# UW-RoboSoccer/tsid_control

Measured on NVIDIA B200. Metric: tsid_qp_ticks_per_sec, higher is better.
Workload: dtype f64

## Files before the change

### tsid_control_b200/csrc/tsidb_kernels.cuh

```cuda
#ifndef TSIDB_KERNELS_CUH_
#define TSIDB_KERNELS_CUH_

#include <cstddef>
#include "tsidb_const.h"

#ifndef TSIDB_EMU
#include <cuda_runtime.h>
#define TSIDB_DEV __device__ __forceinline__
#define TSIDB_HD __host__ __device__
#define TSIDB_DEVNI __device__ __noinline__
__constant__ DevConst g_const[TSIDB_MAX_SLOTS];
#endif

#define FULL 0xffffffffu
#define SCHED_FENCE() asm volatile("" ::: "memory")
#ifdef TSIDB_EMU
#define PHASE_SYNC_D() ((void)0)
#define PHASE_SYNC_E() ((void)0)
#else
#define PHASE_SYNC_D() do { if (TSIDB_LOCK_D) __syncthreads(); } while (0)
#define PHASE_SYNC_E() do { if (TSIDB_LOCK_E) __syncthreads(); } while (0)
#endif
#define TS_EPS 2.220446049250313e-16
#define TS_INF 1.7976931348623157e308
// ... 815 lines not shown
#pragma unroll
      for (int k = 0; k < NV; k++) b[k] = JF[(f * 6 + r) * TSIDB_NVX + k];
    } else if (e < neq) {
      const int u = e - ncm;
#pragma unroll
      for (int k = 0; k < NV; k++) b[k] = Mm[u * SM_LDM + k];
#pragma unroll
      for (int s = 0; s < NC; s++) {
        {
          const int f = (s == 0) ? f0 : 1;
          double jf[6];
#pragma unroll
          for (int r = 0; r < 6; r++) jf[r] = JF[(f * 6 + r) * TSIDB_NVX + u];
#pragma unroll
          for (int o = 0; o < 12; o++) {
            double acc = 0.0;
#pragma unroll
            for (int r = 0; r < 6; r++) acc += C.T[r][o] * jf[r];
            b[NV + 12 * s + o] = -acc;
          }
        }
      }
    } else if (e == neq) {
#pragma unroll
      for (int k = 0; k < N; k++) b[k] = gv[k];
    }
    fwdsub_L<NV, NC>(b, L, ild, C);
    if (e == neq) {
#pragma unroll
      for (int k = 0; k < N; k++) b[k] = -b[k];
    }
    PHASE_SYNC_E();
    auto qr_step = [&](const int i, auto top_tag) {
      constexpr bool top = decltype(top_tag)::value;
      PHASE_SYNC_E();
      const int head = top ? i : NV + (i - ncm);
      __syncwarp();
      if (lane == i) {
        double2* c2 = reinterpret_cast<double2*>(colp);
#pragma unroll
        for (int k = (top ? 0 : ncm); k < (top ? NV : N); k += 2) c2[k >> 1] = make_double2(b[k], b[k + 1]);
      }
      __syncwarp();
      double part = 0.0;
      if (top) {
        if (lane > i && lane < NV) { const double t = colp[lane]; part = t * t; }
      } else {
        for (int k = lane; k < n; k += 32) {
          const bool in_span = (k >= ncm && k < NV) || k > head;
          if (in_span) { const double t = colp[k]; part += t * t; }
        }
      }
      const double sigma = warp_sum(part);
      const double alpha = colp[head];
      const double nrm = sqrt(alpha * alpha + sigma);
      const double beta = (alpha >= 0.0) ? -nrm : nrm;
      if (fabs(beta) <= TS_EPS * R_norm && err == ST_OPTIMAL) err = ST_ERROR;
      R_norm = fmax(R_norm, fabs(beta));
      const double uh = alpha - beta;
      if (top) {
        Vt[i * LDV + lane] = (lane == i) ? uh : ((lane > i && lane < NV) ? colp[lane] : 0.0);
        if (lane + 32 < N) Vt[i * LDV + lane + 32] = 0.0;
      } else {
        for (int k = lane; k < N; k += 32) {
          const bool in_span = (k >= ncm && k < NV) || k > head;
          Vt[i * LDV + k] = (k == head) ? uh : (in_span ? colp[k] : 0.0);
        }
      }
      const double tau = -1.0 / (beta * uh);
      if (lane == 0) { tauq[i] = tau; Rd[i] = beta; }
      __syncwarp();
      if (lane > i && lane <= neq) {
        if (top) reflect<N, 0, NV, (NC == 2)>(b, Vt + i * LDV, tau);
        else reflect<N, ncm, N, (NC == 2)>(b, Vt + i * LDV, tau);
      }
    };
    constexpr int n_top = (nc == 0) ? neq : ncm;
    for (int i = 0; i < n_top; i++) qr_step(i, BoolTag<true>());
    for (int i = n_top; i < neq; i++) qr_step(i, BoolTag<false>());
    __syncwarp();
    if (lane <= neq) {
      store_R1<N, NV, ncm, neq>(R1, b, lane);
    }
    if (lane == neq) {
#pragma unroll
      for (int k = 0; k < N; k++) gv[k] = b[k];
    }
    __syncwarp();
  }
  PHASE_SYNC_E();
  {
    double rhs = 0.0;
    if (lane < ncm) {
      const int s = lane / 6, r = lane % 6;
      const int f = (s == 0) ? f0 : 1;
      rhs = bmot[6 * f + r];
    } else if (lane < neq) {
      rhs = -sm[SE_oNle + lane - ncm];
    }
    const double ird = (lane < neq) ? 1.0 / Rd[lane] : 0.0;
    double accv = rhs * ird;
#pragma unroll
    for (int i = 0; i < neq - 1; i++) {
      const double wi = shfl(accv, i);
      if (lane > i && lane < neq) accv -= (R1[i * SM_LDB + lane] * ird) * wi;
    }
    __syncwarp();
    if (lane < neq) gv[(lane < ncm || nc == 0) ? lane : NV + (lane - ncm)] = accv;
    __syncwarp();
  }
  double y0 = (lane < n) ? gv[lane] : 0.0;
  double y1 = (lane + 32 < n) ? gv[lane + 32] : 0.0;
#pragma unroll
  for (int i = neq - 1; i >= 0; i--) {
    const double v0 = (lane < N) ? Vt[i * LDV + lane] : 0.0;
    const double v1 = (i >= ((nc == 0) ? neq : ncm) && lane + 32 < N) ? Vt[i * LDV + lane + 32] : 0.0;
    const double w = tauq[i] * warp_sum(v0 * y0 + v1 * y1);
    y0 -= w * v0;
    y1 -= w * v1;
  }
  w0v[lane] = y0;
  if (lane + 32 < N) w0v[lane + 32] = y1;
  __syncwarp();
  if (lane < 12 * nc) {
    const int s = lane / 12, i = lane % 12;
    double acc0 = 0.0, acc1 = 0.0;
#pragma unroll
    for (int k = 0; k < 12; k += 2) {
      acc0 += lfinv_sm[k * 12 + i] * w0v[NV + 12 * s + k];
      acc1 += lfinv_sm[(k + 1) * 12 + i] * w0v[NV + 12 * s + k + 1];
    }
    x[NV + lane] = acc0 + acc1;
  }
  {
    const double il = (lane < NV) ? ild[lane] : 0.0;
    y0 *= il;
#pragma unroll
    for (int k = NV - 1; k > 0; k--) {
      const double xk = shfl(y0, k);
      if (lane < k) y0 -= (L[k * SM_LDM + lane] * il) * xk;
    }
  }
  if (lane < NV) x[lane] = y0;
  __syncwarp();
  R_norm_out = R_norm;
  return err;
}

#define SA_LDJA 20
#define SA_LDM 26
struct ALayout {
  int n, m, ldj;
  int oSc, oJ2, oMa, oJFa, oNle, oVj, oX, image;
  int oWr, oR, oNP, oD, oBar, per_env;
};
TSIDB_HD constexpr int even_up(int x) { return (x + 1) & ~1; }
TSIDB_HD constexpr ALayout a_layout(int nv, int nc) {
  ALayout L{};
  const int na = nv - 6;
  L.n = nv + 12 * nc;
  L.m = na + 6 * nc;
  L.ldj = (((L.m / 2) & 1) != 0) ? L.m : L.m + 2;
  L.oSc = 0;
  L.oJ2 = 4;
  L.oMa = L.oJ2 + L.n * L.ldj;
  L.oJFa = L.oMa + na * SA_LDM;
  L.oNle = L.oJFa + 6 * nc * SA_LDJA;
  L.oX = L.oNle + even_up(na);
  L.oVj = L.oX + even_up(L.n);
  L.image = L.oVj + even_up(na);
  L.oWr = L.oVj;
  L.oR = L.oWr + 12;
  L.oNP = L.oR + even_up(L.m * (L.m + 1) / 2);
  L.oD = L.oNP + even_up(L.n);
  L.oBar = L.oD + L.m + 2;
  L.per_env = L.oBar + 2;
  if (L.per_env < L.image + 2) L.per_env = L.image + 2;
  return L;
}
template <int NV, int NC>
struct AL {
  enum : int { n = a_layout(NV, NC).n, m = a_layout(NV, NC).m, ldj = a_layout(NV, NC).ldj, oSc = a_layout(NV, NC).oSc, oJ2 = a_layout(NV, NC).oJ2, oMa = a_layout(NV, NC).oMa, oJFa = a_layout(NV, NC).oJFa, oNle = a_layout(NV, NC).oNle, oVj = a_layout(NV, NC).oVj, oX = a_layout(NV, NC).oX, image = a_layout(NV, NC).image, oWr = a_layout(NV, NC).oWr, oR = a_layout(NV, NC).oR, oNP = a_layout(NV, NC).oNP, oD = a_layout(NV, NC).oD, oBar = a_layout(NV, NC).oBar, per_env = a_layout(NV, NC).per_env };
};
#define SA_IMAGE (a_layout(TSIDB_NVX, 2).image)
#define SA_oSc 0
#define TSIDB_AS_WARPS_DS 8
#define TSIDB_AS_WARPS_SS 12
#define TSIDB_AS_WARPS_FL 12

#ifndef TSIDB_EMU
TSIDB_DEV unsigned smem_u32(const void* p) { return (unsigned)__cvta_generic_to_shared(p); }
TSIDB_DEV void mbar_init(void* bar, int count) {
  asm volatile("mbarrier.init.shared::cta.b64 [%0], %1;" ::"r"(smem_u32(bar)), "r"(count) : "memory");
  asm volatile("fence.mbarrier_init.release.cluster;" ::: "memory");
}
TSIDB_DEV void bulk_load(void* dst, const void* src, unsigned bytes, void* bar) {
  asm volatile("fence.proxy.async.shared::cta;" ::: "memory");
  asm volatile("mbarrier.arrive.expect_tx.shared::cta.b64 _, [%0], %1;" ::"r"(smem_u32(bar)), "r"(bytes) : "memory");
  asm volatile("cp.async.bulk.shared::cluster.global.mbarrier::complete_tx::bytes [%0], [%1], %2, [%3];" ::"r"(smem_u32(dst)),
               "l"(src), "r"(bytes), "r"(smem_u32(bar))
               : "memory");
}
TSIDB_DEV void bulk_store(void* dst, const void* src, unsigned bytes) {
  asm volatile("cp.async.bulk.global.shared::cta.bulk_group [%0], [%1], %2;" ::"l"(dst), "r"(smem_u32(src)), "r"(bytes) : "memory");
}
TSIDB_DEV void bulk_store_commit() { asm volatile("cp.async.bulk.commit_group;" ::: "memory"); }
TSIDB_DEV void bulk_store_wait_read() { asm volatile("cp.async.bulk.wait_group.read 0;" ::: "memory"); }
TSIDB_DEV void bulk_prefetch_l2(const void* src, unsigned bytes) {
  asm volatile("cp.async.bulk.prefetch.L2.global [%0], %1;" ::"l"(src), "r"(bytes) : "memory");
}
TSIDB_DEV void mbar_wait(void* bar, unsigned parity) {
  unsigned ok = 0;
  const unsigned addr = smem_u32(bar);
  do {
    asm volatile("{ .reg .pred p; mbarrier.try_wait.parity.shared::cta.b64 p, [%1], %2; selp.u32 %0, 1, 0, p; }"
                 : "=r"(ok)
                 : "r"(addr), "r"(parity)
                 : "memory");
  } while (!ok);
}
#endif

TSIDB_DEV unsigned long long sortable(double v) {
  unsigned long long b;
  memcpy(&b, &v, 8);
  return (b >> 63) ? ~b : (b | 0x8000000000000000ull);
}
struct LaneConst {
  double lb, ub;
  double tmin, tmax;
  double vmin, vmax;
  double fric[3];
  double Trow[12];
};

struct ASCtx {
  int na, nv;
  int ldj;
  double* J2;
  const double* Ma;
  const double* JFa;
  int nfr;
  int wro;
  const double* nle_a;
  const double* vj;
  double* x;
  double* wr;
  double *Rp, *np, *dd;
};

TSIDB_DEV int fvar0(int nv, int mask, int f) { return nv + ((f == 1 && (mask & 1)) ? 12 : 0); }

#define NRM_LANE0 12
TSIDB_DEV int cid_of(int na, int lane, int slot) {
  return slot == 0 ? lane : (slot == 1 ? 32 + lane - NRM_LANE0 : 36 + (slot - 2) * na + lane);
}
TSIDB_DEV void cid_owner(int na, int cid, int& lane, int& slot) {
  if (cid < 32) { lane = cid; slot = 0; }
  else if (cid < 36) { lane = cid - 32 + NRM_LANE0; slot = 1; }
  else { const int k = cid - 36; slot = 2 + k / na; lane = k - (slot - 2) * na; }
}
TSIDB_DEV int cid_bit(int na, int nv, int cid) {
  if (cid < 32) return 34 * (cid >> 4) + 17 + (cid & 15);
  if (cid < 36) return 34 * ((cid - 32) >> 1) + (((cid - 32) & 1) ? 33 : 16);
  if (cid < 36 + 2 * na) { int k = cid - 36; return 68 + k; }
  int k = cid - 36 - 2 * na;
  int side = k >= na ? 1 : 0, i = k - side * na;
  return 68 + 2 * na + side * nv + 6 + i;
}

TSIDB_DEV void lane_const_init(const DevConst& C, LaneConst& K, int lane) {
  const int na = C.na;
#pragma unroll
  for (int j = 0; j < 12; j++) K.Trow[j] = (lane >= NRM_LANE0 && lane < NRM_LANE0 + 4) ? C.nrm[j % 3] : C.T[lane % 6][j];
#pragma unroll
  for (int j = 0; j < 3; j++) K.fric[j] = C.fric[lane & 3][j];
  K.tmin = (lane < na) ? C.tau_min[lane] : 0.0;
  K.tmax = (lane < na) ? C.tau_max[lane] : 0.0;
  K.vmin = (lane < na) ? C.v_min[lane] : 0.0;
  K.vmax = (lane < na) ? C.v_max[lane] : 0.0;
  K.lb = K.ub = 0.0;
}

TSIDB_DEV void lane_const_load(const double* tables, LaneConst& K, int lane) {
  const double* t = tables + TBL_oLANE + lane;
#pragma unroll
  for (int j = 0; j < 12; j++) K.Trow[j] = t[j * 32];
#pragma unroll
  for (int j = 0; j < 3; j++) K.fric[j] = t[(12 + j) * 32];
  K.tmin = t[15 * 32]; K.tmax = t[16 * 32]; K.vmin = t[17 * 32]; K.vmax = t[18 * 32];
  K.lb = K.ub = 0.0;
}

TSIDB_DEV void eval_rows(const DevConst& C, const ASCtx& S, const LaneConst& K, int lane, int mask, double (&s)[6]) {
  const int na = S.na, nv = S.nv;
  const double* x = S.x;
#pragma unroll
  for (int k = 0; k < 6; k++) s[k] = TS_INF;
  {
    const int f = lane >> 4, c = (lane & 15) >> 2;
    if ((mask >> f) & 1) {
      const double* ff = x + fvar0(nv, mask, f) + 3 * c;
      s[0] = -(K.fric[0] * ff[0] + K.fric[1] * ff[1] + K.fric[2] * ff[2]);
    }
  }
  if (lane < 4) {
    const int f = lane >> 1, side = lane & 1;
    if ((mask >> f) & 1) {
      const double* ff = x + fvar0(nv, mask, f);
      double t = 0.0;
#pragma unroll
      for (int c = 0; c < 4; c++) t += C.nrm[0] * ff[3 * c] + C.nrm[1] * ff[3 * c + 1] + C.nrm[2] * ff[3 * c + 2];
      s[1] = side ? (C.fmax - t) : (t - C.fmin);
    }
  }
  if (lane < na) {
    if (C.use_tb) {
      const double2* Mr = reinterpret_cast<const double2*>(S.Ma + lane * SA_LDM);
      const double2* x2 = reinterpret_cast<const double2*>(x);
      double t0 = S.nle_a[lane], t1 = 0.0, t2 = 0.0, t3 = 0.0;
      int j = 0;
      for (; j + 1 < nv / 2; j += 2) {
        const double2 m0 = Mr[j], m1 = Mr[j + 1], x0 = x2[j], x1 = x2[j + 1];
        t0 += m0.x * x0.x; t1 += m0.y * x0.y; t2 += m1.x * x1.x; t3 += m1.y * x1.y;
      }
      for (; j < nv / 2; j++) { const double2 m0 = Mr[j], x0 = x2[j]; t0 += m0.x * x0.x; t1 += m0.y * x0.y; }
      double u0 = 0.0, u1 = 0.0, u2 = 0.0;
      const double* wb = S.wr + S.wro;
#pragma unroll
      for (int q = 0; q < 12; q += 3) {
        if (q < S.nfr) {
          u0 += S.JFa[q * SA_LDJA + lane] * wb[q];
          u1 += S.JFa[(q + 1) * SA_LDJA + lane] * wb[q + 1];
          u2 += S.JFa[(q + 2) * SA_LDJA + lane] * wb[q + 2];
        }
      }
      const double t = ((t0 + t1) + (t2 + t3)) - ((u0 + u1) + u2);
      s[2] = t - K.tmin;
      s[3] = K.tmax - t;
    }
    if (C.use_jb) {
      s[4] = x[6 + lane] - K.lb;
      s[5] = K.ub - x[6 + lane];
    }
  }
}
TSIDB_DEV double eval_one(const DevConst& C, const ASCtx& S, const LaneConst& K, int cid, int mask) {
  const int na = S.na, nv = S.nv;
  const double* x = S.x;
  if (cid < 32) {
    const int f = cid >> 4, c = (cid & 15) >> 2, k = cid & 3;
    const double* ff = x + fvar0(nv, mask, f) + 3 * c;
    return -(C.fric[k][0] * ff[0] + C.fric[k][1] * ff[1] + C.fric[k][2] * ff[2]);
  }
  if (cid < 36) {
    const int f = (cid - 32) >> 1, side = (cid - 32) & 1;
    const double* ff = x + fvar0(nv, mask, f);
    double t = 0.0;
#pragma unroll
    for (int c = 0; c < 4; c++) t += C.nrm[0] * ff[3 * c] + C.nrm[1] * ff[3 * c + 1] + C.nrm[2] * ff[3 * c + 2];
    return side ? (C.fmax - t) : (t - C.fmin);
  }
  if (cid < 36 + 2 * na) {
    const int k = cid - 36, side = k >= na ? 1 : 0, r = k - side * na;
    const double* Mr = S.Ma + r * SA_LDM;
    double t = S.nle_a[r];
    for (int j = 0; j < nv; j++) t += Mr[j] * x[j];
#pragma unroll
    for (int q = 0; q < 12; q++)
      if (q < S.nfr) t -= S.JFa[q * SA_LDJA + r] * S.wr[S.wro + q];
    return side ? (C.tau_max[r] - t) : (t - C.tau_min[r]);
  }
  {
    const int k = cid - 36 - 2 * na, side = k >= na ? 1 : 0, i = k - side * na;
    const double lim = shfl(side ? K.ub : K.lb, i);
    return side ? lim - x[6 + i] : x[6 + i] - lim;
  }
}

TSIDB_DEV double row_dot_col(const DevConst& C, const ASCtx& S, int cid, int mask, int n, int lane, double* np) {
  const int na = S.na, nv = S.nv;
  const double* Jc = S.J2 + lane;
  if (cid < 32) {
    const int f = cid >> 4, c = (cid & 15) >> 2, k = cid & 3;
    const int r0 = fvar0(nv, mask, f) + 3 * c;
    return -(C.fric[k][0] * Jc[r0 * S.ldj] + C.fric[k][1] * Jc[(r0 + 1) * S.ldj] + C.fric[k][2] * Jc[(r0 + 2) * S.ldj]);
  }
  if (cid < 36) {
    const int f = (cid - 32) >> 1, side = (cid - 32) & 1;
    const int r0 = fvar0(nv, mask, f);
    double t = 0.0;
#pragma unroll
    for (int o = 0; o < 12; o++) t += C.nrm[o % 3] * Jc[(r0 + o) * S.ldj];
    return side ? -t : t;
  }
  if (cid >= 36 + 2 * na) {
    const int k = cid - 36 - 2 * na, side = k >= na ? 1 : 0, i = k - side * na;
    const double t = Jc[(6 + i) * S.ldj];
    return side ? -t : t;
  }
  double d0 = 0.0, d1 = 0.0, d2 = 0.0, d3 = 0.0;
  int k = 0;
  for (; k + 3 < n; k += 4) {
    d0 += np[k] * Jc[k * S.ldj]; d1 += np[k + 1] * Jc[(k + 1) * S.ldj];
    d2 += np[k + 2] * Jc[(k + 2) * S.ldj]; d3 += np[k + 3] * Jc[(k + 3) * S.ldj];
  }
  for (; k < n; k++) d0 += np[k] * Jc[k * S.ldj];
  return (d0 + d1) + (d2 + d3);
}
TSIDB_DEV void actuation_normal(const DevConst& C, const ASCtx& S, int cid, int mask, int n, double* np, int lane) {
  const int na = S.na, nv = S.nv;
  const int q = cid - 36, side = q >= na ? 1 : 0, r = q - side * na;
  for (int k = lane; k < n; k += 32) {
    double val;
    if (k < nv) val = S.Ma[r * SA_LDM + k];
    else {
      const int o = k - nv;
      const int blk = o / 12, j = o % 12;
      double t = 0.0;
#pragma unroll
      for (int kk = 0; kk < 6; kk++) t += C.T[kk][j] * S.JFa[(blk * 6 + kk) * SA_LDJA + r];
      val = -t;
    }
    np[k] = side ? -val : val;
  }
}

TSIDB_DEV double wrench_of(int nv, const LaneConst& K, const double* x, int mask, double* wr, int lane) {
  double s = 0.0;
  if (lane < NRM_LANE0 + 4) {
    const int f = (lane < NRM_LANE0) ? lane / 6 : (lane - NRM_LANE0) >> 1;
    if ((mask >> f) & 1) {
      const double* ff = x + fvar0(nv, mask, f);
      double s0 = 0.0, s1 = 0.0, s2 = 0.0;
#pragma unroll
      for (int j = 0; j < 12; j += 3) { s0 += K.Trow[j] * ff[j]; s1 += K.Trow[j + 1] * ff[j + 1]; s2 += K.Trow[j + 2] * ff[j + 2]; }
      s = (s0 + s1) + s2;
    }
    if (lane < NRM_LANE0) wr[lane] = s;
  }
  return s;
}

TSIDB_DEV int warp_argmin_fast(double val, bool valid, int tiebreak) {
  const unsigned long long key = sortable(val);
  const unsigned hi = valid ? (unsigned)(key >> 32) : 0xffffffffu;
  const unsigned mhi = __reduce_min_sync(FULL, hi);
  const bool v1 = valid && hi == mhi;
  const unsigned b1 = __ballot_sync(FULL, v1);
  if (b1 == 0u) return -1;
  if ((b1 & (b1 - 1u)) == 0u) return __ffs(b1) - 1;
  const unsigned lo = v1 ? (unsigned)key : 0xffffffffu;
  const unsigned mlo = __reduce_min_sync(FULL, lo);
  const bool v2 = v1 && lo == mlo;
  const unsigned tb = v2 ? (unsigned)tiebreak : 0xffffffffu;
  const unsigned mtb = __reduce_min_sync(FULL, tb);
  const unsigned win = __ballot_sync(FULL, v2 && tb == mtb);
  return win ? (__ffs(win) - 1) : -1;
}

template <int NV, int NC>
TSIDB_DEV int as_solve2(const DevConst& C, const ASCtx& S, const LaneConst& K, int lane, int mask, double c1c2, double trH,
                        double R_norm, int& iters_out, uint64_t* act_words, double& lam_out, int& lam_row_out) {
  typedef AL<NV, NC> LA;
  constexpr int nv = NV, na = NV - 6, n = LA::n, m = LA::m, ldj = LA::ldj;
  double* J2 = S.J2;
  double* x = S.x;
  double* wr = S.wr;
  double* Rp = S.Rp;
  double* np = S.np;
  double* dd = S.dd;
  iters_out = 0;
  act_words[0] = act_words[1] = act_words[2] = 0;
  if (lane < 2) dd[m + lane] = 0.0;

  const int nin_ref = C.nin_ref_fixed + 34 * NC;
  const double psi_thresh = (double)nin_ref * TS_EPS * c1c2 * 100.0;
  const int bit_f = 34 * (lane >> 4) + 17 + (lane & 15);
  const int bit_n = 34 * ((lane & 3) >> 1) + ((lane & 1) ? 33 : 16);
  const int bit_a = 68 + lane;
  const int bit_j = 68 + 2 * na + 6 + lane;
  const bool has0 = lane < n, has1 = lane + 32 < n;
  double xr0 = has0 ? x[lane] : 0.0, xr1 = has1 ? x[lane + 32] : 0.0;
  double xo0 = xr0, xo1 = xr1;
  double ur = 0.0, uo = 0.0, irl = 0.0;
  int Ar = 0, Ao = 0;
  int iq = 0, iter = 0, status = ST_OPTIMAL;
  unsigned actbits = 0;
  unsigned exclbits = 0;

  for (;;) {
    iter++;
    if (iter >= C.max_iter) { status = ST_MAX_ITER; break; }
    const double nf = wrench_of(nv, K, x, mask, wr, lane);
    __syncwarp();
    double c0 = TS_INF, c1 = TS_INF, c2 = TS_INF, c3 = TS_INF;
    int side2 = 0, side3 = 0;
    {
      const int f = lane >> 4, c = (lane & 15) >> 2;
      if ((mask >> f) & 1) {
        const double* ff = x + fvar0(nv, mask, f) + 3 * c;
        c0 = -(K.fric[0] * ff[0] + K.fric[1] * ff[1] + K.fric[2] * ff[2]);
      }
    }
    if (lane >= NRM_LANE0 && lane < NRM_LANE0 + 4) {
      const int f = (lane - NRM_LANE0) >> 1, side = lane & 1;
      if ((mask >> f) & 1) c1 = side ? (C.fmax - nf) : (nf - C.fmin);
    }
    if (lane < na) {
      if (C.use_tb) {
        const double2* Mr = reinterpret_cast<const double2*>(S.Ma + lane * SA_LDM);
        const double2* x2 = reinterpret_cast<const double2*>(x);
        double t0 = S.nle_a[lane], t1 = 0.0, t2 = 0.0, t3 = 0.0;
#pragma unroll
        for (int j = 0; j + 1 < nv / 2; j += 2) {
          const double2 m0 = Mr[j], m1 = Mr[j + 1], x0 = x2[j], x1 = x2[j + 1];
          t0 += m0.x * x0.x; t1 += m0.y * x0.y; t2 += m1.x * x1.x; t3 += m1.y * x1.y;
        }
        if ((nv / 2) & 1) { const double2 m0 = Mr[nv / 2 - 1], x0 = x2[nv / 2 - 1]; t0 += m0.x * x0.x; t1 += m0.y * x0.y; }
        double u0 = 0.0, u1 = 0.0, u2 = 0.0;
        const double* wb = wr + S.wro;
#pragma unroll
        for (int q = 0; q < 6 * NC; q += 3) {
          u0 += S.JFa[q * SA_LDJA + lane] * wb[q];
          u1 += S.JFa[(q + 1) * SA_LDJA + lane] * wb[q + 1];
          u2 += S.JFa[(q + 2) * SA_LDJA + lane] * wb[q + 2];
        }
        const double t = ((t0 + t1) + (t2 + t3)) - ((u0 + u1) + u2);
        const double slo = t - K.tmin, sup = K.tmax - t;
        side2 = sup < slo;
        c2 = side2 ? sup : slo;
      }
      if (C.use_jb) {
        const double xv = x[6 + lane];
        const double slo = xv - K.lb, sup = K.ub - xv;
        side3 = sup < slo;
        c3 = side3 ? sup : slo;
      }
    }
    double part = (c0 < 0.0) ? c0 : 0.0;
    part += (c1 < 0.0) ? c1 : 0.0;
    part += (c2 < 0.0) ? c2 : 0.0;
    part += (c3 < 0.0) ? c3 : 0.0;
    exclbits = 0;
    double best;
    int bslot, bbit;
    auto pick = [&]() {
      best = 0.0; bslot = -1; bbit = 1 << 30;
      const unsigned blocked = actbits | exclbits;
      auto consider = [&](double val, int slot, int bit) {
        if (val < 0.0 && !((blocked >> slot) & 1u) && (val < best || (val == best && bit < bbit))) { best = val; bslot = slot; bbit = bit; }
      };
      consider(c0, 0, bit_f);
      consider(c1, 1, bit_n);
      consider(c2, 2 + side2, bit_a + side2 * na);
      consider(c3, 4 + side3, bit_j + side3 * nv);
    };
    pick();
    int src = warp_argmin_fast(best, bslot >= 0, bbit);
    const double psi = warp_sum(part);
    if (fabs(psi) <= psi_thresh) { status = ST_OPTIMAL; break; }
    xo0 = xr0; xo1 = xr1; uo = ur; Ao = Ar;
    bool done = false, restart_l1 = false, first_pick = true;
    for (;;) {
      if (!first_pick) {
        pick();
        src = warp_argmin_fast(best, bslot >= 0, bbit);
      }
      first_pick = false;
      if (src < 0) { status = ST_OPTIMAL; done = true; break; }
      const int ip_slot = __shfl_sync(FULL, bslot, src);
      const int ip = cid_of(na, src, ip_slot);
      double s_ip = shfl(best, src);
      const bool dense_row = (ip_slot == 2 || ip_slot == 3);
#ifdef TSIDB_EMU_TRACE
      if (lane == 0) printf("[emu] iter %d pick bit %d s=%.17g iq=%d\n", iter, cid_bit(na, nv, ip), s_ip, iq);
#endif
      if (dense_row) { actuation_normal(C, S, ip, mask, n, np, lane); __syncwarp(); }
      double up = 0.0;
      for (;;) {
        double dl = 0.0;
        if (lane < m) dl = row_dot_col(C, S, ip, mask, n, lane, np);
        if (lane < m) dd[lane] = (lane >= iq) ? dl : 0.0;
        __syncwarp();
        double z0 = 0.0, z1 = 0.0;
        const double2* Jr0 = reinterpret_cast<const double2*>(J2 + (has0 ? lane : 0) * ldj);
        const double2* Jr1 = reinterpret_cast<const double2*>(J2 + (has1 ? lane + 32 : 0) * ldj);
        if (iq < m) {
          const int cb = iq >> 1;
          constexpr int ce = (m + 1) >> 1;
          const double2* d2 = reinterpret_cast<const double2*>(dd);
          double a0 = 0.0, a1 = 0.0, b0 = 0.0, b1 = 0.0, a2 = 0.0, a3 = 0.0, b2 = 0.0, b3 = 0.0;
#define TSIDB_ZPAIR(c)                                                                       \
  if ((c) < ce) {                                                                            \
    const double2 j0 = Jr0[c], j1 = Jr1[c], dv = d2[c];                                      \
    if ((c) & 1) { a2 += j0.x * dv.x; a3 += j0.y * dv.y; b2 += j1.x * dv.x; b3 += j1.y * dv.y; } \
    else { a0 += j0.x * dv.x; a1 += j0.y * dv.y; b0 += j1.x * dv.x; b1 += j1.y * dv.y; }     \
  }
#define TSIDB_ZSEG(s) if (cb < 4 * (s) + 4 && 4 * (s) < ce) { TSIDB_ZPAIR(4 * (s)) TSIDB_ZPAIR(4 * (s) + 1) TSIDB_ZPAIR(4 * (s) + 2) TSIDB_ZPAIR(4 * (s) + 3) }
          TSIDB_ZSEG(0) TSIDB_ZSEG(1) TSIDB_ZSEG(2) TSIDB_ZSEG(3)
#undef TSIDB_ZSEG
#undef TSIDB_ZPAIR
          static_assert(ce <= 16, "four segments of four column pairs");
          z0 = has0 ? (a0 + a1) + (a2 + a3) : 0.0;
          z1 = has1 ? (b0 + b1) + (b2 + b3) : 0.0;
        }
        double rl;
        {
          double accv = dl * irl;
          const double* col = Rp + (iq - 1) * iq / 2 + lane;
          for (int i = iq - 1; i > 0; i--) {
            const double ri = shfl(accv, i);
            if (lane < i) accv -= (col[0] * irl) * ri;
            col -= i;
          }
          rl = accv;
        }
        double t1 = TS_INF;
        const bool t1_valid = lane < iq && rl > 0.0;
        if (t1_valid) t1 = ur / rl;
        const int lpos = (__ballot_sync(FULL, t1_valid) != 0u) ? warp_argmin_fast(t1, t1_valid, lane) : -1;
        t1 = (lpos >= 0) ? shfl(t1, lpos) : TS_INF;
        const double d2sum = warp_sum((lane >= iq && lane < m) ? dl * dl : 0.0);
        bool z_nonzero = d2sum > 64.0 * TS_EPS * trH;
        if (!z_nonzero) z_nonzero = fabs(warp_sum(z0 * z0 + z1 * z1)) > TS_EPS;
        const double t2 = z_nonzero ? (-s_ip / d2sum) : TS_INF;
        const double t = fmin(t1, t2);
#ifdef TSIDB_EMU_TRACE
        if (lane == 0) printf("[emu]   t1=%.17g (pos %d) t2=%.17g znp=%.6g\n", t1, lpos, t2, d2sum);
#endif
        if (t >= TS_INF) { status = ST_INFEASIBLE; done = true; break; }
        if (lane < iq) ur -= t * rl;
        up += t;
        if (t2 < TS_INF) {
          xr0 += t * z0;
          xr1 += t * z1;
          if (has0) x[lane] = xr0;
          if (has1) x[lane + 32] = xr1;
        }
        if (t2 < TS_INF && t == t2) {
          bool degenerate = true;
          if (iq < m) {
            const double nrm = sqrt(d2sum);
            const double d0 = shfl(dl, iq);
            const double beta = (d0 >= 0.0) ? -nrm : nrm;
            degenerate = !(fabs(beta) > TS_EPS * R_norm);
            if (!degenerate) {
              const double rho = 1.0 / (beta * (d0 - beta));
              if (lane == iq) dd[iq] = d0 - beta;
              const double w0 = has0 ? -rho * (z0 - beta * J2[lane * ldj + iq]) : 0.0;
              const double w1 = has1 ? -rho * (z1 - beta * J2[(lane + 32) * ldj + iq]) : 0.0;
              __syncwarp();
              {
                const int cb = iq >> 1;
                constexpr int ce = (m + 1) >> 1;
                const double2* v2 = reinterpret_cast<const double2*>(dd);
                double2* W0 = const_cast<double2*>(Jr0);
                double2* W1 = const_cast<double2*>(Jr1);
#define TSIDB_HSEG(s)                                                                                          \
  if (cb < 4 * (s) + 4 && 4 * (s) < ce) {                                                                      \
    constexpr int c_ = 4 * (s);                                                                                \
    double2 vq[4], p0[4], p1[4];                                                                               \
    _Pragma("unroll") for (int k = 0; k < 4; k++) if (c_ + k < ce) { vq[k] = v2[c_ + k]; p0[k] = Jr0[c_ + k]; p1[k] = Jr1[c_ + k]; } \
    _Pragma("unroll") for (int k = 0; k < 4; k++) if (c_ + k < ce) {                                           \
      p0[k].x -= w0 * vq[k].x; p0[k].y -= w0 * vq[k].y; p1[k].x -= w1 * vq[k].x; p1[k].y -= w1 * vq[k].y;       \
    }                                                                                                          \
    _Pragma("unroll") for (int k = 0; k < 4; k++) if (c_ + k < ce) { if (has0) W0[c_ + k] = p0[k]; if (has1) W1[c_ + k] = p1[k]; } \
  }
                TSIDB_HSEG(0) TSIDB_HSEG(1) TSIDB_HSEG(2) TSIDB_HSEG(3)
#undef TSIDB_HSEG
              }
              if (lane < iq) Rp[iq * (iq + 1) / 2 + lane] = dl;
              if (lane == iq) { Rp[iq * (iq + 1) / 2 + iq] = beta; irl = rho * (d0 - beta); ur = up; Ar = ip; }
              R_norm = fmax(R_norm, fabs(beta));
              if (lane == src) actbits |= 1u << ip_slot;
              iq++;
              __syncwarp();
            }
          }
#ifdef TSIDB_EMU_TRACE
          if (lane == 0) printf("[emu]   add -> %s Rnorm=%.6g\n", degenerate ? "DEGENERATE" : "ok", R_norm);
#endif
          if (degenerate) {
            if (lane == src) exclbits |= 1u << ip_slot;
            actbits = 0;
            if (lane < iq) { Ar = Ao; ur = uo; }
            xr0 = xo0; xr1 = xo1;
            if (has0) x[lane] = xr0;
            if (has1) x[lane + 32] = xr1;
            __syncwarp();
            for (int i = 0; i < iq; i++) {
// ... 204 lines not shown
    const double2* s0 = reinterpret_cast<const double2*>(sm + SM_oH);
    double2* d0 = reinterpret_cast<double2*>(eimg + SE_oH);
    for (int k = lane; k < (702 + TSIDB_NX) / 2; k += 32) d0[k] = s0[k];
    const double2* s1 = reinterpret_cast<const double2*>(sm + SM_oJF);
    double2* d1 = reinterpret_cast<double2*>(eimg + SE_oJF);
    for (int k = lane; k < 312 / 2; k += 32) d1[k] = s1[k];
  } else if (lane == 0) {
    asm volatile("fence.proxy.async.shared::cta;" ::: "memory");
    bulk_store(eimg + SE_oH, sm + SM_oH, (702 + TSIDB_NX) * sizeof(double));
    bulk_store(eimg + SE_oJF, sm + SM_oJF, 312 * sizeof(double));
    bulk_store_commit();
  }
#else
  for (int k = lane; k < 702; k += 32) eimg[SE_oH + k] = sm[SM_oH + k];
  for (int k = lane; k < TSIDB_NX; k += 32) eimg[SE_oG + k] = sm[SM_oGv + k];
  for (int k = lane; k < 312; k += 32) eimg[SE_oJF + k] = sm[SM_oJF + k];
#endif
  if (lane < 8) eimg[SE_oNle + lane] = (lane < 6) ? sm[SM_oNle + lane] : 0.0;
  if (lane < 12) eimg[SE_oBm + lane] = sm[SM_oBv + BV_MOT + lane];
  if (lane < 2) eimg[SE_oSc + lane] = (lane == 0) ? (double)mask : 0.0;
  __syncwarp();
}

template <int NV, int NC>
TSIDB_DEV void j2_from_factor(const DevConst& C, const double* L, const double* ild, const double* tauq, const double* Vt,
                              double* img, int lane);
template <int NV, int NC, bool LOCAL = false>
TSIDB_DEV void eliminate_env(const DevConst& C, const double* lfinv_sm, double* sm, const TickArgs& a, int slot, int lane, unsigned& parity) {
  typedef EL<NV, NC> LE;
  __syncwarp();
#ifndef TSIDB_EMU
  if (!LOCAL) {
    if (lane == 0) bulk_load(sm, a.ws3 + (size_t)slot * SE_IMAGE, SE_IMAGE * sizeof(double), sm + LE::oBar);
    mbar_wait(sm + LE::oBar, parity);
    parity ^= 1u;
  }
#else
  for (int k = lane; k < SE_IMAGE; k += 32) sm[k] = a.ws3[(size_t)slot * SE_IMAGE + k];
#endif
  __syncwarp();
  const int mask = (int)sm[SE_oSc];
  constexpr int n = NV + 12 * NC;
  double c1c2 = 0.0, c1 = 0.0, R_norm = 1.0;
  const int err = k3_eliminate<NV, NC>(C, lfinv_sm, sm, lane, mask, c1c2, c1, R_norm);
  typedef AL<NV, NC> LA;
  double* img = a.ws + (size_t)slot * SA_IMAGE;
  for (int k = lane; k < even_up(n); k += 32) img[LA::oX + k] = (k < n) ? sm[LE::oX + k] : 0.0;
  if (lane == 0) { img[SA_oSc] = c1c2; img[SA_oSc + 1] = R_norm; img[SA_oSc + 2] = (double)(4 * err + mask); img[SA_oSc + 3] = c1; }
  __syncwarp();
  if (err == ST_OPTIMAL) j2_from_factor<NV, NC>(C, sm + SE_oH, sm + LE::oILD, sm + LE::oTAU, sm + LE::oVT, img, lane);
  __syncwarp();
}

template <int NV, int NC>
TSIDB_DEV void j2_from_factor(const DevConst& C, const double* L, const double* ild, const double* tauq, const double* Vt,
                              double* img, int lane) {
  constexpr int N = NV + 12 * NC, NEQ = 6 + 6 * NC, NCM = 6 * NC, M = N - NEQ;
  constexpr int NS = N;
  typedef AL<NV, NC> LA;
  if (lane >= M) return;
  double q[N];
#pragma unroll
  for (int k = 0; k < N; k++) {
    const int col = (NC == 0) ? k - 6 : ((k < NV) ? k - NCM : ((k >= NV + 6) ? (NV - NCM) + (k - NV - 6) : -1));
    q[k] = (col >= 0 && col == lane) ? 1.0 : 0.0;
  }
#pragma unroll
  for (int i = NEQ - 1; i >= 0; i--) {
    const bool top = (i < NCM) || NC == 0;
    const int head = top ? i : NV + (i - NCM);
    const int lo = top ? i + 1 : NCM;
    const int flo = top ? N : head + 1;
    const double2* v2 = reinterpret_cast<const double2*>(Vt + i * NS);
    double w0 = 0.0, w1 = 0.0, w2 = 0.0, w3 = 0.0;
#pragma unroll
    for (int kk = (lo & ~1); kk < NV; kk += 2) {
      const double2 p = v2[kk >> 1];
      if (kk >= lo) { if (kk & 2) w2 += p.x * q[kk]; else w0 += p.x * q[kk]; }
      if (kk & 2) w3 += p.y * q[kk + 1]; else w1 += p.y * q[kk + 1];
    }
#pragma unroll
    for (int kk = (flo & ~1); kk < N; kk += 2) {
      const double2 p = v2[kk >> 1];
      if (kk >= flo) { if (kk & 2) w2 += p.x * q[kk]; else w0 += p.x * q[kk]; }
      if (kk & 2) w3 += p.y * q[kk + 1]; else w1 += p.y * q[kk + 1];
    }
    const double w = tauq[i] * ((w0 + w1) + (w2 + w3));
    q[head] = -w * Vt[i * NS + head];
#pragma unroll
    for (int kk = (lo & ~1); kk < NV; kk += 2) {
      const double2 p = v2[kk >> 1];
      if (kk >= lo) q[kk] -= w * p.x;
      q[kk + 1] -= w * p.y;
    }
#pragma unroll
    for (int kk = (flo & ~1); kk < N; kk += 2) {
      const double2 p = v2[kk >> 1];
      if (kk >= flo) q[kk] -= w * p.x;
      q[kk + 1] -= w * p.y;
    }
    if (i == NCM) {
#pragma unroll
      for (int s = 0; s < NC; s++) {
#pragma unroll
        for (int r = 0; r < 12; r++) {
          double acc = 0.0;
#pragma unroll
          for (int k = r; k < 12; k++) acc += C.Lfinv[k][r] * q[NV + 12 * s + k];
          img[LA::oJ2 + (NV + 12 * s + r) * LA::ldj + lane] = acc;
        }
      }
    }
  }
#pragma unroll
  for (int k = NV - 1; k >= 0; k--) {
    q[k] *= ild[k];
    const int i0 = (k * SM_LDM) & 1;
    if (i0 && k > 0) q[0] -= L[k * SM_LDM] * q[k];
#pragma unroll
    for (int ii = i0; ii < k; ii += 2) {
      if (ii + 1 < k) {
        const double2 p = *reinterpret_cast<const double2*>(L + k * SM_LDM + ii);
        q[ii] -= p.x * q[k];
        q[ii + 1] -= p.y * q[k];
      } else {
        q[ii] -= L[k * SM_LDM + ii] * q[k];
      }
    }
  }
#pragma unroll
  for (int k = 0; k < NV; k++) img[LA::oJ2 + k * LA::ldj + lane] = q[k];
}

template <int NV, int NC, bool LOCAL = false>
TSIDB_DEV void activeset_env(const DevConst& C, LaneConst& K, double* sm, const TickArgs& a, int env, int slot, int lane, unsigned& parity) {
  typedef AL<NV, NC> LA;
  constexpr int nv = NV, na = NV - 6;
  __syncwarp();
#ifndef TSIDB_EMU
  if (!LOCAL) {
    if (lane == 0) bulk_load(sm, a.ws + (size_t)slot * SA_IMAGE, LA::image * sizeof(double), sm + LA::oBar);
    mbar_wait(sm + LA::oBar, parity);
    parity ^= 1u;
  }
#else
  for (int k = lane; k < LA::image; k += 32) sm[k] = a.ws[(size_t)slot * SA_IMAGE + k];
#endif
  __syncwarp();
  ASCtx S;
  S.na = na; S.nv = nv; S.ldj = LA::ldj; S.nfr = 6 * NC;
  S.J2 = sm + LA::oJ2; S.Ma = sm + LA::oMa; S.JFa = sm + LA::oJFa; S.nle_a = sm + LA::oNle; S.vj = sm + LA::oVj;
  S.x = sm + LA::oX; S.wr = sm + LA::oWr;
  S.Rp = sm + LA::oR; S.np = sm + LA::oNP; S.dd = sm + LA::oD;
  const double c1c2 = sm[SA_oSc], R_norm = sm[SA_oSc + 1], c1 = sm[SA_oSc + 3];
  const int em = (int)sm[SA_oSc + 2], err = em >> 2, mask = em & 3;
  S.wro = (NC == 1 && !(mask & 1)) ? 6 : 0;
  K.lb = K.ub = 0.0;
  if (lane < na && C.use_jb) {
    const double vj = S.vj[lane];
    K.ub = fmin((K.vmax - vj) / C.jb_dt, 1e10);
    K.lb = fmax((K.vmin - vj) / C.jb_dt, -1e10);
  }
  __syncwarp();
  int iters = 0;
  uint64_t words[3] = {0, 0, 0};
  int status = err;
  double lam = 0.0;
  int lam_row = -1;
  if (err == ST_OPTIMAL) status = as_solve2<NV, NC>(C, S, K, lane, mask, c1c2, c1, R_norm, iters, words, lam, lam_row);
  const bool ok = (status == ST_OPTIMAL || status == ST_MAX_ITER);
  const double* x = S.x;
  double* wr = S.wr;
  if (ok) wrench_of(nv, K, x, mask, wr, lane);
  __syncwarp();
  if (lane < nv) a.ddq[eidx(a, env, lane, nv)] = ok ? x[lane] : 0.0;
  if (lane < 24) {
    const int f = lane / 12;
    double val = 0.0;
    if (ok && ((mask >> f) & 1)) val = x[fvar0(nv, mask, f) + lane % 12];
    a.f[eidx(a, env, lane, 24)] = val;
  }
  if (lane < na) {
    double val = 0.0;
    if (ok) {
      const double* Mr = S.Ma + lane * SA_LDM;
      double s0 = S.nle_a[lane], s1 = 0.0;
      for (int j = 0; j < nv; j += 2) { s0 += Mr[j] * x[j]; s1 += (j + 1 < nv) ? Mr[j + 1] * x[j + 1] : 0.0; }
      double s = s0 + s1;
#pragma unroll
      for (int q = 0; q < 6 * NC; q++) s -= S.JFa[q * SA_LDJA + lane] * wr[S.wro + q];
      val = s;
    }
    a.tau[eidx(a, env, lane, na)] = val;
  }
  if (a.o_wrench && lane < 12) a.o_wrench[eidx(a, env, lane, 12)] = ok ? wr[lane] : 0.0;
  if (a.o_lambda) a.o_lambda[(size_t)env * 32 + lane] = lam;
  if (a.o_lambda_row) a.o_lambda_row[(size_t)env * 32 + lane] = lam_row;
  if (lane == 0) {
    a.status[env] = status;
    a.iters[env] = iters;
    if (a.pred) a.pred[env] = iters;
    if (a.active) {
      a.active[env] = words[0];
      a.active[(size_t)a.n_envs + env] = words[1];
      a.active[2 * (size_t)a.n_envs + env] = words[2];
    }
  }
  __syncwarp();
}

template <int NV>
struct PB {
  enum : int {
    oE = 0,
    oMa = SE_IMAGE,
    oNle = oMa + (NV - 6) * SA_LDM,
    oVj = oNle + even_up(NV - 6),
    oJc = oVj + even_up(NV - 6),
    per_env = oJc + NV * 24
  };
};
TSIDB_DEV void st_pair(double* p, double x, double y) { *reinterpret_cast<double2*>(p) = make_double2(x, y); }

TSIDB_DEV int ci_block(const DevConst& C, int ri, int nc, int na, int nv, int& side, int& i, int& slot) {
  int r = ri;
  for (int s = 0; s < nc; s++) {
    if (r < 34) { slot = s; side = r >= 17; i = r - 17 * side; return 0; }
    r -= 34;
  }
  if (C.use_tb) {
    if (r < 2 * na) { side = r >= na; i = r - na * side; return 2; }
    r -= 2 * na;
  }
  if (C.use_jb && r < 2 * nv) { side = r >= nv; i = r - nv * side; return 3; }
  return -1;
}

template <int NV>
TSIDB_DEV void problem_env(const DevConst& C, const double* pt, double* sm, const TickArgs& a, const ProblemOut& o, int env,
                           int lane) {
  typedef PB<NV> P;
  constexpr int nv = NV, na = NV - 6, NX = NV + 24, NEQX = 18;
  const double BIG = 1e10;
  const int nin_x = 2 * (34 + (C.use_tb ? na : 0) + (C.use_jb ? nv : 0));
  __syncwarp();
  {
    const double2* s = reinterpret_cast<const double2*>(a.ws3 + (size_t)env * SE_IMAGE);
    double2* d = reinterpret_cast<double2*>(sm + P::oE);
    for (int k = lane; k < SE_IMAGE / 2; k += 32) d[k] = s[k];
  }
  const int mask = a.mask ? (a.mask[env] & 3) : 3;
  const int nc = (mask & 1) + ((mask >> 1) & 1);
  const int n = nv + 12 * nc, neq = 6 + 6 * nc;
  const int nin = 2 * (17 * nc + (C.use_tb ? na : 0) + (C.use_jb ? nv : 0));
  const int f0 = (mask & 1) ? 0 : 1;
  {
    const ALayout L = a_layout(nv, nc);
    const double* img = a.ws + (size_t)env * SA_IMAGE;
    const double2* s = reinterpret_cast<const double2*>(img + L.oMa);
    double2* d = reinterpret_cast<double2*>(sm + P::oMa);
    for (int k = lane; k < na * SA_LDM / 2; k += 32) d[k] = s[k];
    if (lane < na) { sm[P::oNle + lane] = img[L.oNle + lane]; sm[P::oVj + lane] = img[L.oVj + lane]; }
  }
  __syncwarp();
  const double* E = sm + P::oE;
  const double* Ma = sm + P::oMa;
  double* Jc = sm + P::oJc;
  if (lane < nv) {
    for (int s = 0; s < nc; s++) {
      const int f = s == 0 ? f0 : 1;
      double jf[6];
#pragma unroll
      for (int m = 0; m < 6; m++) jf[m] = E[SE_oJF + (f * 6 + m) * TSIDB_NVX + lane];
#pragma unroll
      for (int k = 0; k < 12; k++) {
        double acc = 0.0;
#pragma unroll
        for (int m = 0; m < 6; m++) acc += pt[PT_oT + m * 12 + k] * jf[m];
        Jc[lane * 24 + 12 * s + k] = acc;
      }
    }
  }
  __syncwarp();
  const bool cols = lane < NX / 2;
  if (o.H && cols) {
    double* out = o.H + (size_t)env * NX * NX + 2 * lane;
    for (int i = 0; i < NX; i++) {
      double x[2];
#pragma unroll
      for (int u = 0; u < 2; u++) {
        const int j = 2 * lane + u;
        double val = 0.0;
        if (i < n && j < n) {
          if (i < nv && j < nv) val = E[SE_oH + (i >= j ? i * SM_LDM + j : j * SM_LDM + i)];
          else if (i >= nv && j >= nv && (i - nv) / 12 == (j - nv) / 12) val = pt[PT_oHF + ((i - nv) % 12) * 12 + (j - nv) % 12];
        }
        x[u] = val;
      }
      st_pair(out + i * NX, x[0], x[1]);
    }
  }
  if (o.g)
    for (int k = lane; k < NX; k += 32) o.g[(size_t)env * NX + k] = k < nv ? E[SE_oG + k] : 0.0;
  if (o.CE && cols) {
    double* out = o.CE + (size_t)env * NEQX * NX + 2 * lane;
    for (int r = 0; r < NEQX; r++) {
// ... 1034 lines not shown
```

Measured before the change: 21.01 million.

## Skip torque-bound row evaluation when iterate change provably cannot violate bounds

Adds per-lane norm bounds on the torque-constraint rows, computed once before the active-set loop. Each iteration then uses a warp-wide maximum of how far x has moved since the last exact evaluation to decide whether any torque-bound row could have become violated. If none could, the Ma·x and JFa·w dot products are skipped. This adds setup work, warp reductions and shared-memory state (xa, kb, lr) to save repeated per-iteration matrix-vector work, at the cost of relying on a conservative floating-point bound with small safety margins.

```diff
diff --git a/tsid_control_b200/csrc/tsidb_kernels.cuh b/tsid_control_b200/csrc/tsidb_kernels.cuh
--- a/tsid_control_b200/csrc/tsidb_kernels.cuh
+++ b/tsid_control_b200/csrc/tsidb_kernels.cuh
@@ -991,7 +991,7 @@
 struct ALayout {
   int n, m, ldj;
   int oSc, oJ2, oMa, oJFa, oNle, oVj, oX, image;
-  int oWr, oR, oNP, oD, oBar, per_env;
+  int oWr, oR, oNP, oD, oXa, oKb, oLr, oBar, per_env;
 };
 TSIDB_HD constexpr int even_up(int x) { return (x + 1) & ~1; }
 TSIDB_HD constexpr ALayout a_layout(int nv, int nc) {
@@ -1012,14 +1012,17 @@
   L.oR = L.oWr + 12;
   L.oNP = L.oR + even_up(L.m * (L.m + 1) / 2);
   L.oD = L.oNP + even_up(L.n);
-  L.oBar = L.oD + L.m + 2;
+  L.oXa = L.oD + L.m + 2;
+  L.oKb = L.oXa + even_up(L.n);
+  L.oLr = L.oKb + even_up(na);
+  L.oBar = L.oLr + even_up(na);
   L.per_env = L.oBar + 2;
   if (L.per_env < L.image + 2) L.per_env = L.image + 2;
   return L;
 }
 template <int NV, int NC>
 struct AL {
-  enum : int { n = a_layout(NV, NC).n, m = a_layout(NV, NC).m, ldj = a_layout(NV, NC).ldj, oSc = a_layout(NV, NC).oSc, oJ2 = a_layout(NV, NC).oJ2, oMa = a_layout(NV, NC).oMa, oJFa = a_layout(NV, NC).oJFa, oNle = a_layout(NV, NC).oNle, oVj = a_layout(NV, NC).oVj, oX = a_layout(NV, NC).oX, image = a_layout(NV, NC).image, oWr = a_layout(NV, NC).oWr, oR = a_layout(NV, NC).oR, oNP = a_layout(NV, NC).oNP, oD = a_layout(NV, NC).oD, oBar = a_layout(NV, NC).oBar, per_env = a_layout(NV, NC).per_env };
+  enum : int { n = a_layout(NV, NC).n, m = a_layout(NV, NC).m, ldj = a_layout(NV, NC).ldj, oSc = a_layout(NV, NC).oSc, oJ2 = a_layout(NV, NC).oJ2, oMa = a_layout(NV, NC).oMa, oJFa = a_layout(NV, NC).oJFa, oNle = a_layout(NV, NC).oNle, oVj = a_layout(NV, NC).oVj, oX = a_layout(NV, NC).oX, image = a_layout(NV, NC).image, oWr = a_layout(NV, NC).oWr, oR = a_layout(NV, NC).oR, oNP = a_layout(NV, NC).oNP, oD = a_layout(NV, NC).oD, oXa = a_layout(NV, NC).oXa, oKb = a_layout(NV, NC).oKb, oLr = a_layout(NV, NC).oLr, oBar = a_layout(NV, NC).oBar, per_env = a_layout(NV, NC).per_env };
 };
 #define SA_IMAGE (a_layout(TSIDB_NVX, 2).image)
 #define SA_oSc 0
@@ -1086,6 +1089,7 @@
   double* x;
   double* wr;
   double *Rp, *np, *dd;
+  double *xa, *kb, *lr;
 };
 
 TSIDB_DEV int fvar0(int nv, int mask, int f) { return nv + ((f == 1 && (mask & 1)) ? 12 : 0); }
@@ -1281,6 +1285,22 @@
   return s;
 }
 
+TSIDB_DEV double warp_max_bound(unsigned hi) {
+  const unsigned m = ~__reduce_min_sync(FULL, ~hi);
+  if (m >= 0x7ff00000u) return TS_INF;
+  const unsigned long long b = (unsigned long long)(m + 1u) << 32;
+  double v;
+  memcpy(&v, &b, 8);
+  return v;
+}
+TSIDB_DEV unsigned hi_word(double v) {
+  unsigned long long b;
+  memcpy(&b, &v, 8);
+  return (unsigned)(b >> 32);
+}
+#ifndef TSIDB_AS_PATH_COUNT
+#define TSIDB_AS_PATH_COUNT(lane, exact) ((void)0)
+#endif
 TSIDB_DEV int warp_argmin_fast(double val, bool valid, int tiebreak) {
   const unsigned long long key = sortable(val);
   const unsigned hi = valid ? (unsigned)(key >> 32) : 0xffffffffu;
@@ -1327,6 +1347,34 @@
   int iq = 0, iter = 0, status = ST_OPTIMAL;
   unsigned actbits = 0;
   unsigned exclbits = 0;
+  double thr = -TS_INF;
+  if (C.use_tb && lane < na) {
+    const double* Mr = S.Ma + lane * SA_LDM;
+    double m1 = 0.0, f1 = 0.0, j1 = 0.0, t1max = 0.0;
+    for (int j = 0; j < nv; j++) m1 += fabs(Mr[j]);
+#pragma unroll
+    for (int q = 0; q < 6 * NC; q++) j1 += fabs(S.JFa[q * SA_LDJA + lane]);
+#pragma unroll 1
+    for (int kk = 0; kk < 6; kk++) {
+      double t1 = 0.0;
+#pragma unroll
+      for (int j = 0; j < 12; j++) t1 += fabs(C.T[kk][j]);
+      t1max = fmax(t1max, t1);
+    }
+#pragma unroll 1
+    for (int j = 0; j < 12; j++) {
+#pragma unroll
+      for (int blk = 0; blk < NC; blk++) {
+        double t = 0.0;
+#pragma unroll
+        for (int kk = 0; kk < 6; kk++) t += C.T[kk][j] * S.JFa[(blk * 6 + kk) * SA_LDJA + lane];
+        f1 += fabs(t);
+      }
+    }
+    const double lr = m1 + j1 * t1max;
+    S.kb[lane] = (m1 + f1) + 1e-10 * lr;
+    S.lr[lane] = lr;
+  }
 
   for (;;) {
     iter++;
@@ -1346,36 +1394,48 @@
       const int f = (lane - NRM_LANE0) >> 1, side = lane & 1;
       if ((mask >> f) & 1) c1 = side ? (C.fmax - nf) : (nf - C.fmin);
     }
-    if (lane < na) {
-      if (C.use_tb) {
-        const double2* Mr = reinterpret_cast<const double2*>(S.Ma + lane * SA_LDM);
-        const double2* x2 = reinterpret_cast<const double2*>(x);
-        double t0 = S.nle_a[lane], t1 = 0.0, t2 = 0.0, t3 = 0.0;
-#pragma unroll
-        for (int j = 0; j + 1 < nv / 2; j += 2) {
-          const double2 m0 = Mr[j], m1 = Mr[j + 1], x0 = x2[j], x1 = x2[j + 1];
-          t0 += m0.x * x0.x; t1 += m0.y * x0.y; t2 += m1.x * x1.x; t3 += m1.y * x1.y;
+    if (C.use_tb) {
+      const unsigned h0 = has0 ? hi_word(fabs(xr0 - S.xa[lane])) : 0u, h1 = has1 ? hi_word(fabs(xr1 - S.xa[lane + 32])) : 0u;
+      const double emax = warp_max_bound(h0 > h1 ? h0 : h1);
+      const bool cleared = lane >= na || thr > S.kb[lane] * emax;
+      const bool exact = __ballot_sync(FULL, !cleared) != 0u;
+      TSIDB_AS_PATH_COUNT(lane, exact);
+      if (exact) {
+        if (lane < na) {
+          const double2* Mr = reinterpret_cast<const double2*>(S.Ma + lane * SA_LDM);
+          const double2* x2 = reinterpret_cast<const double2*>(x);
+          double t0 = S.nle_a[lane], t1 = 0.0, t2 = 0.0, t3 = 0.0;
+#pragma unroll
+          for (int j = 0; j + 1 < nv / 2; j += 2) {
+            const double2 m0 = Mr[j], m1 = Mr[j + 1], x0 = x2[j], x1 = x2[j + 1];
+            t0 += m0.x * x0.x; t1 += m0.y * x0.y; t2 += m1.x * x1.x; t3 += m1.y * x1.y;
+          }
+          if ((nv / 2) & 1) { const double2 m0 = Mr[nv / 2 - 1], x0 = x2[nv / 2 - 1]; t0 += m0.x * x0.x; t1 += m0.y * x0.y; }
+          double u0 = 0.0, u1 = 0.0, u2 = 0.0;
+          const double* wb = wr + S.wro;
+#pragma unroll
+          for (int q = 0; q < 6 * NC; q += 3) {
+            u0 += S.JFa[q * SA_LDJA + lane] * wb[q];
+            u1 += S.JFa[(q + 1) * SA_LDJA + lane] * wb[q + 1];
+            u2 += S.JFa[(q + 2) * SA_LDJA + lane] * wb[q + 2];
+          }
+          const double t = ((t0 + t1) + (t2 + t3)) - ((u0 + u1) + u2);
+          const double slo = t - K.tmin, sup = K.tmax - t;
+          side2 = sup < slo;
+          c2 = side2 ? sup : slo;
         }
-        if ((nv / 2) & 1) { const double2 m0 = Mr[nv / 2 - 1], x0 = x2[nv / 2 - 1]; t0 += m0.x * x0.x; t1 += m0.y * x0.y; }
-        double u0 = 0.0, u1 = 0.0, u2 = 0.0;
-        const double* wb = wr + S.wro;
-#pragma unroll
-        for (int q = 0; q < 6 * NC; q += 3) {
-          u0 += S.JFa[q * SA_LDJA + lane] * wb[q];
-          u1 += S.JFa[(q + 1) * SA_LDJA + lane] * wb[q + 1];
-          u2 += S.JFa[(q + 2) * SA_LDJA + lane] * wb[q + 2];
-        }
-        const double t = ((t0 + t1) + (t2 + t3)) - ((u0 + u1) + u2);
-        const double slo = t - K.tmin, sup = K.tmax - t;
-        side2 = sup < slo;
-        c2 = side2 ? sup : slo;
-      }
-      if (C.use_jb) {
-        const double xv = x[6 + lane];
-        const double slo = xv - K.lb, sup = K.ub - xv;
-        side3 = sup < slo;
-        c3 = side3 ? sup : slo;
-      }
+        if (has0) S.xa[lane] = xr0;
+        if (has1) S.xa[lane + 32] = xr1;
+        const unsigned g0 = hi_word(fabs(xr0)), g1 = hi_word(fabs(xr1));
+        const double xn = warp_max_bound(g0 > g1 ? g0 : g1);
+        if (lane < na) thr = c2 - 1e-10 * (fabs(S.nle_a[lane]) + fmax(fabs(K.tmin), fabs(K.tmax)) + S.lr[lane] * xn);
+      }
+    }
+    if (lane < na && C.use_jb) {
+      const double xv = x[6 + lane];
+      const double slo = xv - K.lb, sup = K.ub - xv;
+      side3 = sup < slo;
+      c3 = side3 ? sup : slo;
     }
     double part = (c0 < 0.0) ? c0 : 0.0;
     part += (c1 < 0.0) ? c1 : 0.0;
@@ -1886,6 +1946,7 @@
   S.J2 = sm + LA::oJ2; S.Ma = sm + LA::oMa; S.JFa = sm + LA::oJFa; S.nle_a = sm + LA::oNle; S.vj = sm + LA::oVj;
   S.x = sm + LA::oX; S.wr = sm + LA::oWr;
   S.Rp = sm + LA::oR; S.np = sm + LA::oNP; S.dd = sm + LA::oD;
+  S.xa = sm + LA::oXa; S.kb = sm + LA::oKb; S.lr = sm + LA::oLr;
   const double c1c2 = sm[SA_oSc], R_norm = sm[SA_oSc + 1], c1 = sm[SA_oSc + 3];
   const int em = (int)sm[SA_oSc + 2], err = em >> 2, mask = em & 3;
   S.wro = (NC == 1 && !(mask & 1)) ? 6 : 0;
```

New measurement: 20.53 million (median of 6 runs). 0.977x the previous value.
